# Quantus-Network/qp-zk-circuits

Measured on AMD Instinct MI355X. Metric: Wormhole proofs/sec, higher is better.
Workload: dtype u64

## Files before the change

### qp-zk-circuits_amd/csrc/poseidon.hpp

```cpp
#pragma once
#include <stddef.h>
#include "gl64.hpp"

namespace poseidon {
using gl::u32;
using gl::u64;

constexpr int WIDTH = 12, RATE = 8, HALF_FULL = 4, PARTIAL = 22, ROUNDS = 30;

GL_HD u64 sbox7(u64 x) {
    u64 x2 = gl::sqr(x), x4 = gl::sqr(x2), x3 = gl::mul(x, x2);
    return gl::mul(x3, x4);
}
#if defined(__HIP_DEVICE_COMPILE__) && defined(POSEIDON_GROUPED_SBOX)
template <int N>
__device__ __forceinline__ void sbox7_layer(u64 (&x)[N]) {
    u64 x2[N], x3[N], x4[N];
    gl::mul_group(x2, x, x);
    gl::mul_group(x4, x2, x2);
    gl::mul_group(x3, x, x2);
    gl::mul_group(x, x3, x4);
}
__device__ __forceinline__ u64 sbox7_lane(u64 x) {
    u64 a[1] = {x}, x2[1];
    gl::mul_group(x2, a, a);
    u64 l[2] = {x2[0], x}, r[2] = {x2[0], x2[0]}, q[2];
    gl::mul_group(q, l, r);
    u64 c[1] = {q[0]}, d[1] = {q[1]}, o[1];
    gl::mul_group(o, c, d);
    return o[0];
}
#else
template <int N>
GL_HD void sbox7_layer(u64 (&x)[N]) {
#if defined(__HIP_DEVICE_COMPILE__)
#pragma unroll
#endif
    for (int i = 0; i < N; i++) x[i] = sbox7(x[i]);
}
GL_HD u64 sbox7_lane(u64 x) { return sbox7(x); }
#endif

GL_HD void mds_layer_naive(u64 (&s)[WIDTH]) {
    constexpr u32 C[WIDTH] = {17, 15, 41, 16, 2, 28, 13, 13, 39, 18, 34, 20};
    u32 lo[WIDTH], hi[WIDTH];
#pragma unroll
    for (int i = 0; i < WIDTH; i++) { lo[i] = (u32)s[i]; hi[i] = (u32)(s[i] >> 32); }
#pragma unroll
    for (int r = 0; r < WIDTH; r++) {
        u64 al = 0, ah = 0;
#pragma unroll
        for (int i = 0; i < WIDTH; i++) {
            const int j = (i + r) % WIDTH;
            al += (u64)lo[j] * C[i];
            ah += (u64)hi[j] * C[i];
        }
        if (r == 0) { al += (u64)lo[0] * 8u; ah += (u64)hi[0] * 8u; }
        u64 low = al + (ah << 32);
        u32 top = (u32)(ah >> 32) + (low < al ? 1u : 0u);
        s[r] = gl::reduce96(low, top);
    }
}

typedef long long i64;
GL_HD i64 shl(i64 x, int k) { return (i64)((u64)x << k); }
GL_HD void mds_circulant_half(const i64 (&x)[WIDTH], i64 (&o)[WIDTH]) {
    i64 U1[3], Um[3], F[3], H[3];
#pragma unroll
    for (int b = 0; b < 3; b++) {
        const i64 e = x[b] + x[b + 6], f = x[b] - x[b + 6], g = x[b + 3] + x[b + 9], h = x[b + 3] - x[b + 9];
        U1[b] = e + g; Um[b] = e - g; F[b] = f; H[b] = h;
    }
    const i64 T = U1[0] + U1[1] + U1[2];
    const i64 A[3] = {T + U1[2], T + U1[0], T + U1[1]};
    const i64 B[3] = {shl(Um[2], 3) - Um[0] - shl(Um[1], 1),
                      -(shl(Um[0], 3) + Um[1] + shl(Um[2], 1)),
                      shl(Um[0], 1) - shl(Um[1], 3) - Um[2]};
    const i64 f0 = F[0], f1 = F[1], f2 = F[2], h0 = H[0], h1 = H[1], h2 = H[2];
    const i64 R[3] = {shl(f0, 1) - h0 + f1 - shl(h1, 4) + f2 + shl(h2, 2),
                      -shl(f0, 2) + h0 + shl(f1, 1) - h1 + f2 - shl(h2, 4),
                      shl(f0, 4) + h0 - shl(f1, 2) + h1 + shl(f2, 1) - h2};
    const i64 I[3] = {f0 + shl(h0, 1) + shl(f1, 4) + h1 - shl(f2, 2) + h2,
                      -f0 - shl(h0, 2) + f1 + shl(h1, 1) + shl(f2, 4) + h2,
                      -f0 + shl(h0, 4) - f1 - shl(h1, 2) + f2 + shl(h2, 1)};
#pragma unroll
    for (int b = 0; b < 3; b++) {
        const i64 a16 = shl(A[b], 4), p = a16 + B[b], q = a16 - B[b];
        o[b] = p + R[b]; o[b + 3] = q + I[b]; o[b + 6] = p - R[b]; o[b + 9] = q - I[b];
    }
}

template <int FIRST, int COUNT>
GL_HD void mds_layer_rows(u64 (&s)[WIDTH]) {
    static_assert(FIRST >= 0 && COUNT >= 1 && FIRST + COUNT <= WIDTH, "rows of the state");
    i64 lo[WIDTH], hi[WIDTH], ol[WIDTH], oh[WIDTH];
#pragma unroll
    for (int i = 0; i < WIDTH; i++) { lo[i] = (i64)(u32)s[i]; hi[i] = (i64)(s[i] >> 32); }
    mds_circulant_half(lo, ol);
    mds_circulant_half(hi, oh);
    ol[0] += shl(lo[0], 3); oh[0] += shl(hi[0], 3);
#pragma unroll
    for (int r = FIRST; r < FIRST + COUNT; r++) {
        const u64 al = (u64)ol[r], ah = (u64)oh[r];
        const u64 low = al + (ah << 32);
        const u32 top = (u32)(ah >> 32) + (low < al ? 1u : 0u);
        s[r] = gl::reduce96(low, top);
    }
}
GL_HD void mds_layer(u64 (&s)[WIDTH]) { mds_layer_rows<0, WIDTH>(s); }

struct Spectrum { i64 U1[3], Um[3], F[3], H[3]; };
GL_HD void spectrum_of(const i64 (&x)[WIDTH], Spectrum &s) {
#pragma unroll
    for (int b = 0; b < 3; b++) {
        const i64 e = x[b] + x[b + 6], g = x[b + 3] + x[b + 9];
        s.U1[b] = e + g; s.Um[b] = e - g; s.F[b] = x[b] - x[b + 6]; s.H[b] = x[b + 3] - x[b + 9];
    }
}
GL_HD void spectrum_times_circulant(Spectrum &s) {
    const i64 T = s.U1[0] + s.U1[1] + s.U1[2];
    const i64 A0 = T + s.U1[2], A1 = T + s.U1[0], A2 = T + s.U1[1];
    const i64 B0 = shl(s.Um[2], 3) - s.Um[0] - shl(s.Um[1], 1);
    const i64 B1 = -(shl(s.Um[0], 3) + s.Um[1] + shl(s.Um[2], 1));
    const i64 B2 = shl(s.Um[0], 1) - shl(s.Um[1], 3) - s.Um[2];
    const i64 f0 = s.F[0], f1 = s.F[1], f2 = s.F[2], h0 = s.H[0], h1 = s.H[1], h2 = s.H[2];
    const i64 R0 = shl(f0, 1) - h0 + f1 - shl(h1, 4) + f2 + shl(h2, 2);
    const i64 R1 = -shl(f0, 2) + h0 + shl(f1, 1) - h1 + f2 - shl(h2, 4);
    const i64 R2 = shl(f0, 4) + h0 - shl(f1, 2) + h1 + shl(f2, 1) - h2;
    const i64 I0 = f0 + shl(h0, 1) + shl(f1, 4) + h1 - shl(f2, 2) + h2;
    const i64 I1 = -f0 - shl(h0, 2) + f1 + shl(h1, 1) + shl(f2, 4) + h2;
    const i64 I2 = -f0 + shl(h0, 4) - f1 - shl(h1, 2) + f2 + shl(h2, 1);
    s.U1[0] = shl(A0, 6); s.U1[1] = shl(A1, 6); s.U1[2] = shl(A2, 6);
    s.Um[0] = shl(B0, 2); s.Um[1] = shl(B1, 2); s.Um[2] = shl(B2, 2);
    s.F[0] = shl(R0, 1); s.F[1] = shl(R1, 1); s.F[2] = shl(R2, 1);
    s.H[0] = shl(I0, 1); s.H[1] = shl(I1, 1); s.H[2] = shl(I2, 1);
}
GL_HD i64 spectrum_lane0(const Spectrum &s) { return (s.U1[0] + s.Um[0] + shl(s.F[0], 1)) >> 2; }
GL_HD void vector_of(const Spectrum &s, i64 (&x)[WIDTH]) {
#pragma unroll
    for (int b = 0; b < 3; b++) {
        const i64 p = s.U1[b] + s.Um[b], q = s.U1[b] - s.Um[b], f2 = shl(s.F[b], 1), h2 = shl(s.H[b], 1);
        x[b] = (p + f2) >> 2; x[b + 6] = (p - f2) >> 2; x[b + 3] = (q + h2) >> 2; x[b + 9] = (q - h2) >> 2;
    }
}
GL_HD u64 join_halves(i64 lo, i64 hi) {
    const u64 al = (u64)lo, ah = (u64)hi;
    const u64 low = al + (ah << 32);
    const u32 top = (u32)(ah >> 32) + (low < al ? 1u : 0u);
    return gl::reduce96(low, top);
}
GL_HD void renormalize_pair(i64 &lo, i64 &hi) {
    const i64 k = (lo >> 32) & ~(i64)3;
    lo -= shl(k, 32); hi += k;
    const i64 m = (hi >> 32) & ~(i64)3;
    hi -= shl(m, 32); hi += m; lo -= m;
}
GL_HD void renormalize(Spectrum &sl, Spectrum &sh) {
#pragma unroll
    for (int b = 0; b < 3; b++) {
        renormalize_pair(sl.U1[b], sh.U1[b]); renormalize_pair(sl.Um[b], sh.Um[b]);
        renormalize_pair(sl.F[b], sh.F[b]); renormalize_pair(sl.H[b], sh.H[b]);
    }
}
GL_HD u64 join_signed_halves(i64 lo, i64 hi) { return join_halves(lo + (((i64)1 << 60) + ((i64)1 << 28)), hi + (((i64)1 << 60) - ((i64)1 << 29))); }

GL_HD void partial_rounds_spectral(u64 (&s)[WIDTH], const u64 *rc0) {
    i64 lo[WIDTH], hi[WIDTH];
#pragma unroll
    for (int i = 0; i < WIDTH; i++) { lo[i] = (i64)(u32)s[i]; hi[i] = (i64)(s[i] >> 32); }
    Spectrum sl, sh;
    spectrum_of(lo, sl); spectrum_of(hi, sh);
    i64 x_lo = lo[0], x_hi = hi[0];
    i64 d_lo = 0, d_hi = 0;
    u64 x0 = s[0];
#pragma unroll 1
    for (int k0 = 0; k0 < PARTIAL; k0 += 3) {
#pragma unroll
        for (int kk = 0; kk < 3; kk++) {
            const int k = k0 + kk;
            if (k < PARTIAL) {
                if (k) x0 = join_signed_halves(x_lo + d_lo, x_hi + d_hi);
                const u64 y = sbox7_lane(gl::add_canonical(x0, rc0[k * WIDTH]));
                const i64 y_lo = (i64)(u32)y, y_hi = (i64)(y >> 32);
                const i64 in_lo = y_lo - x_lo, in_hi = y_hi - x_hi;
                sl.U1[0] += in_lo; sl.Um[0] += in_lo; sl.F[0] += in_lo;
                sh.U1[0] += in_hi; sh.Um[0] += in_hi; sh.F[0] += in_hi;
                spectrum_times_circulant(sl); spectrum_times_circulant(sh);
                d_lo = shl(y_lo, 3); d_hi = shl(y_hi, 3);
                if (kk == 2 && k + 1 < PARTIAL) renormalize(sl, sh);
                x_lo = spectrum_lane0(sl); x_hi = spectrum_lane0(sh);
            }
        }
    }
    vector_of(sl, lo); vector_of(sh, hi);
    lo[0] += d_lo; hi[0] += d_hi;
#pragma unroll
    for (int i = 0; i < WIDTH; i++) s[i] = join_signed_halves(lo[i], hi[i]);
}

GL_HD void permute(u64 (&s)[WIDTH], const u64 *rc) {
    int r = 0;
    for (int k = 0; k < HALF_FULL; k++, r++) {
#pragma unroll
        for (int i = 0; i < WIDTH; i++) s[i] = gl::add_canonical(s[i], rc[r * WIDTH + i]);
        sbox7_layer(s);
        mds_layer(s);
    }
#pragma unroll
    for (int i = 1; i < WIDTH; i++) s[i] = gl::add_canonical(s[i], rc[r * WIDTH + i]);
    partial_rounds_spectral(s, rc + r * WIDTH);
    r += PARTIAL;
    for (int k = 0; k < HALF_FULL; k++, r++) {
#pragma unroll
        for (int i = 0; i < WIDTH; i++) s[i] = gl::add_canonical(s[i], rc[r * WIDTH + i]);
        sbox7_layer(s);
        mds_layer(s);
    }
#pragma unroll
    for (int i = 0; i < WIDTH; i++) s[i] = gl::canon(s[i]);
}
GL_HD void permute_layerwise(u64 (&s)[WIDTH], const u64 *rc) {
    int r = 0;
    for (int k = 0; k < HALF_FULL; k++, r++) {
#pragma unroll
        for (int i = 0; i < WIDTH; i++) s[i] = sbox7(gl::add_canonical(s[i], rc[r * WIDTH + i]));
        mds_layer(s);
    }
#pragma unroll
    for (int i = 1; i < WIDTH; i++) s[i] = gl::add_canonical(s[i], rc[r * WIDTH + i]);
    for (int k = 0; k < PARTIAL; k++, r++) {
        s[0] = sbox7(gl::add_canonical(s[0], rc[r * WIDTH]));
        mds_layer(s);
    }
    for (int k = 0; k < HALF_FULL; k++, r++) {
#pragma unroll
        for (int i = 0; i < WIDTH; i++) s[i] = sbox7(gl::add_canonical(s[i], rc[r * WIDTH + i]));
        mds_layer(s);
    }
#pragma unroll
    for (int i = 0; i < WIDTH; i++) s[i] = gl::canon(s[i]);
}
GL_HD void permute_textbook(u64 (&s)[WIDTH], const u64 *rc) {
    int r = 0;
    for (int k = 0; k < ROUNDS; k++, r++) {
        const bool full = k < HALF_FULL || k >= HALF_FULL + PARTIAL;
        for (int i = 0; i < WIDTH; i++) s[i] = gl::add_canonical(s[i], rc[r * WIDTH + i]);
        for (int i = 0; i < (full ? WIDTH : 1); i++) s[i] = sbox7(s[i]);
        mds_layer_naive(s);
    }
    for (int i = 0; i < WIDTH; i++) s[i] = gl::canon(s[i]);
}

constexpr int FP_FIRST = 0, FP_RC = 12, FP_VS = 34, FP_WHATS = FP_VS + 22 * 11, FP_INIT = FP_WHATS + 22 * 11, FP_WORDS = FP_INIT + 121;
constexpr u64 MDS_00 = 25;

GL_HD void fast_partial_enter(u64 (&s)[WIDTH], const u64 *fp) {
#pragma unroll
    for (int i = 0; i < WIDTH; i++) s[i] = gl::add(s[i], fp[FP_FIRST + i]);
    u64 t[11];
    for (int c = 0; c < 11; c++) {
        u64 acc = 0;
        for (int r = 0; r < 11; r++) acc = gl::add(acc, gl::mul(fp[FP_INIT + c * 11 + r], s[1 + r]));
        t[c] = acc;
    }
    for (int c = 0; c < 11; c++) s[1 + c] = t[c];
}
GL_HD void fast_partial_linear(u64 (&s)[WIDTH], const u64 *fp, int r) {
    const u64 s0 = gl::add(s[0], fp[FP_RC + r]);
    u64 d = gl::mul(s0, MDS_00);
    for (int i = 0; i < 11; i++) d = gl::add(d, gl::mul(fp[FP_WHATS + r * 11 + i], s[1 + i]));
    for (int i = 0; i < 11; i++) s[1 + i] = gl::add(s[1 + i], gl::mul(s0, fp[FP_VS + r * 11 + i]));
    s[0] = d;
}
const u64 *host_fast_partial();

void derive_round_constants(u64 *out360);
const u64 *host_round_constants();
const u64 *host_hash_round_constants();

}

namespace poseidon2 {
using gl::u64;
struct Params {
    u64 rc_ext[8 * 12];
    u64 rc_int[22];
    u64 diag_m1[12];
    u64 m4[16];
};
constexpr int PARAM_WORDS = 96 + 22 + 12 + 16;
const Params &qp_params();

GL_HD void ext_layer(u64 (&s)[12], const Params &p) {
    u64 t[12];
#pragma unroll
    for (int b = 0; b < 3; b++)
#pragma unroll
        for (int i = 0; i < 4; i++) {
            u64 acc = 0;
#pragma unroll
            for (int j = 0; j < 4; j++) acc = gl::add(acc, gl::mul(p.m4[4 * i + j], s[4 * b + j]));
            t[4 * b + i] = acc;
        }
#pragma unroll
    for (int i = 0; i < 4; i++) {
        const u64 sum = gl::add(gl::add(t[i], t[4 + i]), t[8 + i]);
#pragma unroll
        for (int b = 0; b < 3; b++) s[4 * b + i] = gl::add(t[4 * b + i], sum);
    }
}
GL_HD void ext_layer_qp(u64 (&s)[12]) {
    u64 t[12];
#pragma unroll
    for (int b = 0; b < 3; b++) {
        const u64 a = s[4 * b], bb = s[4 * b + 1], c = s[4 * b + 2], d = s[4 * b + 3];
        const u64 sum = gl::add(gl::add(a, bb), gl::add(c, d));
        t[4 * b] = gl::add(gl::add(sum, a), gl::add(bb, bb));
        t[4 * b + 1] = gl::add(gl::add(sum, bb), gl::add(c, c));
        t[4 * b + 2] = gl::add(gl::add(sum, c), gl::add(d, d));
        t[4 * b + 3] = gl::add(gl::add(sum, d), gl::add(a, a));
    }
#pragma unroll
    for (int i = 0; i < 4; i++) {
        const u64 sum = gl::add(gl::add(t[i], t[4 + i]), t[8 + i]);
#pragma unroll
        for (int b = 0; b < 3; b++) s[4 * b + i] = gl::add(t[4 * b + i], sum);
    }
}
GL_HD void int_layer(u64 (&s)[12], const Params &p) {
    u64 sum = 0;
#pragma unroll
    for (int i = 0; i < 12; i++) sum = gl::add(sum, s[i]);
#pragma unroll
    for (int i = 0; i < 12; i++) s[i] = gl::add(gl::mul(s[i], p.diag_m1[i]), sum);
}
GL_HD void permute_qp(u64 (&s)[12], const Params &p) {
    ext_layer_qp(s);
    for (int r = 0; r < 4; r++) {
#pragma unroll
        for (int i = 0; i < 12; i++) s[i] = gl::add_canonical(s[i], p.rc_ext[r * 12 + i]);
        poseidon::sbox7_layer(s);
        ext_layer_qp(s);
    }
    for (int r = 0; r < 22; r++) {
        s[0] = poseidon::sbox7_lane(gl::add_canonical(s[0], p.rc_int[r]));
        int_layer(s, p);
    }
    for (int r = 4; r < 8; r++) {
#pragma unroll
        for (int i = 0; i < 12; i++) s[i] = gl::add_canonical(s[i], p.rc_ext[r * 12 + i]);
        poseidon::sbox7_layer(s);
        ext_layer_qp(s);
    }
#pragma unroll
    for (int i = 0; i < 12; i++) s[i] = gl::canon(s[i]);
}
GL_HD void permute(u64 (&s)[12], const Params &p) {
    ext_layer(s, p);
    for (int r = 0; r < 4; r++) {
#pragma unroll
        for (int i = 0; i < 12; i++) s[i] = gl::add(s[i], p.rc_ext[r * 12 + i]);
        poseidon::sbox7_layer(s);
        ext_layer(s, p);
    }
    for (int r = 0; r < 22; r++) {
        s[0] = poseidon::sbox7_lane(gl::add(s[0], p.rc_int[r]));
        int_layer(s, p);
    }
    for (int r = 4; r < 8; r++) {
#pragma unroll
        for (int i = 0; i < 12; i++) s[i] = gl::add(s[i], p.rc_ext[r * 12 + i]);
        poseidon::sbox7_layer(s);
        ext_layer(s, p);
    }
#pragma unroll
    for (int i = 0; i < 12; i++) s[i] = gl::canon(s[i]);
}
}

namespace hasher {
enum Kind : int { POSEIDON = 0, POSEIDON2 = 1 };
struct Config {
    int kind = POSEIDON;
    poseidon2::Params p2{};
    void permute(gl::u64 (&s)[12]) const;
};
const Config &process_default();
void set_process_default(int kind, const poseidon2::Params *p);
inline int kind() { return process_default().kind; }
inline void host_permute(gl::u64 (&s)[12]) { process_default().permute(s); }
inline void hash_no_pad(const Config &h, const gl::u64 *in, size_t n, gl::u64 out[4]) {
    gl::u64 st[12] = {0};
    for (size_t i = 0; i < n; i += 8) {
        for (size_t k = 0; k < 8 && i + k < n; k++) st[k] = gl::canon(in[i + k]);
        h.permute(st);
    }
    for (int i = 0; i < 4; i++) out[i] = st[i];
}
}
```

### qp-zk-circuits_amd/csrc/poseidon_mfma.hpp

```cpp
#pragma once
#include <string.h>
#include <utility>
#include "poseidon.hpp"

namespace pmf {
using gl::u32;
using gl::u64;
#if defined(__HIPCC__)
typedef int v4i __attribute__((ext_vector_type(4)));
typedef int v16i __attribute__((ext_vector_type(16)));
#endif

constexpr int LIMBS = 8, N_GROUP = 6, N_FIN = 3, FIN_STEPS = 9, N_ELEM = 36;
constexpr int group_steps(int g) { return 3 + g; }
constexpr int group_base(int g) { int b = 0; for (int i = 0; i < g; i++) b += group_steps(i); return b; }
constexpr int N_GROUP_TILES = group_base(N_GROUP);
constexpr int N_TILES = N_GROUP_TILES + N_FIN * FIN_STEPS;
constexpr int CINIT_OFF = N_TILES * 1024;
constexpr int G_OFF = CINIT_OFF + (N_GROUP + N_FIN) * 128;
constexpr int TABLE_BYTES = G_OFF + 32;
static_assert(N_GROUP_TILES == 33 && TABLE_BYTES % 16 == 0, "table layout");
constexpr u64 DIGIT_BIAS = 0x8080808080808080ull;

constexpr u64 mds_entry(int r, int j) {
    constexpr u32 C[12] = {17, 15, 41, 16, 2, 28, 13, 13, 39, 18, 34, 20};
    return C[(j - r + 12) % 12] + ((r == 0 && j == 0) ? 8 : 0);
}
constexpr u64 small_g(int d) {
    u64 R[12] = {1, 0, 0, 0, 0, 0, 0, 0, 0, 0, 0, 0};
    for (int it = 0; it < d; it++) {
        u64 T[12] = {};
        for (int j = 1; j < 12; j++)
            for (int i = 0; i < 12; i++) T[j] += R[i] * mds_entry(i, j);
        for (int j = 0; j < 12; j++) R[j] = T[j];
    }
    u64 g = 0;
    for (int i = 0; i < 12; i++) g += R[i] * mds_entry(i, 0);
    return g;
}
constexpr u32 G0 = (u32)small_g(0), G1 = (u32)small_g(1), G2 = (u32)small_g(2);
static_assert(small_g(0) == 25 && small_g(1) < small_g(2) && small_g(2) < (1ull << 21), "group coefficients: the bound of reduce96_terms");

GL_HD u64 to_digits(u64 v) {
    u64 t = v + DIGIT_BIAS;
    t += (t < v) ? 0xFFFFFFFFull : 0ull;
    return t ^ DIGIT_BIAS;
}
GL_HD u32 byte_perm(u32 s0, u32 s1, u32 sel) {
#if defined(__HIP_DEVICE_COMPILE__)
    return __builtin_amdgcn_perm(s0, s1, sel);
#else
    const u64 pool = ((u64)s0 << 32) | s1;
    u32 r = 0;
    for (int i = 0; i < 4; i++) r |= (u32)((pool >> (8 * ((sel >> (8 * i)) & 7))) & 0xFF) << (8 * i);
    return r;
#endif
}
GL_HD void recombine_wide(const u32 (&z)[LIMBS], u64 &lo, u32 &top) {
    const u32 a0 = (z[3] << 24) | z[0], a1 = byte_perm(z[6], z[3], 0x05040201u), a2 = z[6] >> 16;
    const u32 b0 = z[1] << 8, b1 = (z[7] << 24) | z[4], b2 = z[7] >> 8;
    const u32 c0 = z[2] << 16, c1 = byte_perm(z[5], z[2], 0x06050402u);
    typedef unsigned __int128 u128;
    const u128 A = ((u128)a2 << 64) | ((u128)a1 << 32) | a0;
    const u128 B = ((u128)b2 << 64) | ((u128)b1 << 32) | b0;
    const u128 Cc = ((u128)c1 << 32) | c0;
    const u128 S = A + B + Cc;
    lo = (u64)S; top = (u32)(S >> 64);
}
GL_HD u64 recombine(const u32 (&z)[LIMBS]) {
    u64 lo; u32 top;
    recombine_wide(z, lo, top);
    return gl::reduce96(lo, top);
}
constexpr int MAX_GROUP_TERMS = 3;
GL_HD u64 reduce96_terms(u64 lo, u32 top, const u64 *y, const u32 *g, int n) {
    if (n == 0) return gl::reduce96(lo, top);
    u64 al = (u32)lo, ah = ((u64)top << 32) | (lo >> 32);
#if defined(__HIP_DEVICE_COMPILE__)
#pragma unroll
#endif
    for (int i = 0; i < n; i++) { al += (u64)(u32)y[i] * g[i]; ah += (y[i] >> 32) * g[i]; }
    const u64 low = al + (ah << 32);
    return gl::reduce96(low, (u32)(ah >> 32) + (low < al ? 1u : 0u));
}
constexpr int row_of(int output, int limb) { const int i = 8 * (output & 1) + limb; return (i & 3) + 8 * (i >> 2) + 4 * (output >> 1); }

#if !defined(__HIP_DEVICE_COMPILE__)
namespace host {
typedef unsigned __int128 u128;
inline u64 fmul(u64 a, u64 b) { return (u64)((u128)a * b % gl::P); }
inline u64 fadd(u64 a, u64 b) { return (u64)(((u128)a + b) % gl::P); }
inline u64 fsub(u64 a, u64 b) { return (u64)(((u128)a + gl::P - b % gl::P) % gl::P); }
inline bool const_digits(u64 w, signed char (&d)[LIMBS]) {
    w %= gl::P;
    __int128 rep = w <= 0x7F7F7F7F7F7F7F7Full ? (__int128)w : (__int128)w - (__int128)gl::P;
    for (int a = 0; a < LIMBS; a++) {
        int dg = (int)(rep & 255);
        if (dg >= 128) dg -= 256;
        d[a] = (signed char)dg;
        rep = (rep - dg) / 256;
    }
    return rep == 0;
}
struct Rows { u64 w[4][N_ELEM]; u64 addc[4]; };
inline bool fill_tiles(const Rows &rw, int steps, unsigned char *tiles, unsigned char *cinit) {
    static signed char dig[4][N_ELEM][8][LIMBS];
    for (int o = 0; o < 4; o++)
        for (int e = 0; e < N_ELEM; e++) {
            u64 w = rw.w[o][e] % gl::P;
            for (int b = 0; b < 8; b++) { if (!const_digits(w, dig[o][e][b])) return false; w = fmul(w, 256); }
        }
    for (int q = 0; q < steps; q++)
        for (int o = 0; o < 4; o++)
            for (int limb = 0; limb < LIMBS; limb++)
                for (int k = 0; k < 32; k++) {
                    const int lane = row_of(o, limb) + 32 * (k >> 4), j = k & 15, e = 4 * q + (k >> 3), b = k & 7;
                    tiles[(size_t)q * 1024 + lane * 16 + j] = (unsigned char)dig[o][e][b][limb];
                }
    u64 bias = 0, pw = 1u << 23;
    for (int l = 0; l < LIMBS; l++) { bias = fadd(bias, pw); pw = fmul(pw, 256); }
    for (int h = 0; h < 2; h++)
        for (int i = 0; i < 16; i++) {
            const u64 c = fsub(rw.addc[2 * h + (i >> 3)], bias);
            const u32 v = (1u << 23) + (u32)((c >> (8 * (i & 7))) & 0xFF);
            memcpy(cinit + h * 64 + i * 4, &v, 4);
        }
    return true;
}
struct Linear {
    u64 M[12][12], pre[12][12];
    u64 rc[22][12], after[12];
};
inline bool build_tables(const Linear &L, unsigned char *tab) {
    static u64 R[23][12], G[22], Q[22][12], NP[12][12];
    const auto &M = L.M;
    for (int j = 0; j < 12; j++) R[0][j] = j == 0;
    for (int k = 0; k < 22; k++)
        for (int j = 0; j < 12; j++) {
            u64 a = 0;
            if (j >= 1) for (int i = 0; i < 12; i++) a = fadd(a, fmul(R[k][i], M[i][j]));
            R[k + 1][j] = a;
        }
    for (int d = 0; d < 22; d++) { u64 a = 0; for (int i = 0; i < 12; i++) a = fadd(a, fmul(R[d][i], M[i][0])); G[d] = a; }
    for (int i = 0; i < 12; i++) Q[0][i] = M[i][0] % gl::P;
    for (int d = 0; d + 1 < 22; d++)
        for (int i = 0; i < 12; i++) { u64 a = 0; for (int j = 1; j < 12; j++) a = fadd(a, fmul(M[i][j], Q[d][j])); Q[d + 1][i] = a; }
    for (int i = 0; i < 12; i++) for (int j = 0; j < 12; j++) NP[i][j] = i == j;
    for (int it = 0; it < 22; it++) {
        u64 T[12][12];
        for (int i = 0; i < 12; i++) for (int e = 0; e < 12; e++) { u64 a = 0; for (int j = 1; j < 12; j++) a = fadd(a, fmul(M[i][j], NP[j][e])); T[i][e] = a; }
        memcpy(NP, T, sizeof T);
    }
    static u64 accv[23][12];
    memset(accv, 0, sizeof accv);
    for (int k = 0; k < 22; k++)
        for (int i = 0; i < 12; i++) { u64 a = 0; for (int j = 1; j < 12; j++) a = fadd(a, fmul(M[i][j], fadd(accv[k][j], L.rc[k][j] % gl::P))); accv[k + 1][i] = a; }
    memset(tab, 0, TABLE_BYTES);
    for (int g = 0; g < N_GROUP; g++) {
        Rows rw{};
        for (int o = 0; o < 4; o++) {
            const int k = 4 * g + o;
            if (k >= 22) continue;
            for (int e = 0; e < 12; e++) { u64 a = 0; for (int i = 0; i < 12; i++) a = fadd(a, fmul(R[k][i], L.pre[i][e])); rw.w[o][e] = a; }
            for (int j = 0; j < 4 * g; j++) rw.w[o][12 + j] = G[k - 1 - j];
            rw.addc[o] = fadd(accv[k][0], L.rc[k][0] % gl::P);
        }
        if (!fill_tiles(rw, group_steps(g), tab + (size_t)group_base(g) * 1024, tab + CINIT_OFF + g * 128)) return false;
    }
    for (int f = 0; f < N_FIN; f++) {
        Rows rw{};
        for (int o = 0; o < 4; o++) {
            const int i = 4 * f + o;
            for (int e = 0; e < 12; e++) { u64 a = 0; for (int j = 0; j < 12; j++) a = fadd(a, fmul(NP[i][j], L.pre[j][e])); rw.w[o][e] = a; }
            for (int j = 0; j < 22; j++) rw.w[o][12 + j] = Q[21 - j][i];
            rw.addc[o] = fadd(accv[22][i], L.after[i] % gl::P);
        }
        if (!fill_tiles(rw, FIN_STEPS, tab + (size_t)(N_GROUP_TILES + f * FIN_STEPS) * 1024, tab + CINIT_OFF + (N_GROUP + f) * 128)) return false;
    }
    memcpy(tab + G_OFF, G, 3 * sizeof(u64));
    return true;
}
inline bool build_tables(const u64 *rc, unsigned char *tab) {
    static Linear L;
    memset(&L, 0, sizeof L);
    for (int r = 0; r < 12; r++) for (int j = 0; j < 12; j++) L.M[r][j] = L.pre[r][j] = mds_entry(r, j);
    for (int k = 0; k < 22; k++) L.rc[k][0] = rc[(4 + k) * 12];
    for (int i = 1; i < 12; i++) L.rc[0][i] = rc[4 * 12 + i];
    for (int i = 0; i < 12; i++) L.after[i] = rc[26 * 12 + i];
    if (!build_tables(L, tab)) return false;
    u64 g[3]; memcpy(g, tab + G_OFF, sizeof g);
    return g[0] == G0 && g[1] == G1 && g[2] == G2;
}
inline bool build_tables_gate(const u64 *rcp, unsigned char *tab) {
    static Linear L;
    memset(&L, 0, sizeof L);
    for (int r = 0; r < 12; r++) for (int j = 0; j < 12; j++) L.M[r][j] = L.pre[r][j] = mds_entry(r, j);
    for (int k = 0; k < 22; k++) for (int i = 0; i < 12; i++) L.rc[k][i] = rcp[(4 + k) * 12 + i];
    for (int i = 0; i < 12; i++) L.after[i] = rcp[26 * 12 + i];
    return build_tables(L, tab);
}
inline bool build_tables_p2(const poseidon2::Params &p, unsigned char *tab) {
    static Linear L;
    memset(&L, 0, sizeof L);
    for (int j = 0; j < 12; j++) {
        u64 e[12] = {}, f[12] = {};
        e[j] = f[j] = 1;
        poseidon2::int_layer(e, p); poseidon2::ext_layer_qp(f);
        for (int i = 0; i < 12; i++) { L.M[i][j] = gl::canon(e[i]); L.pre[i][j] = gl::canon(f[i]); }
    }
    for (int k = 0; k < 22; k++) L.rc[k][0] = p.rc_int[k];
    for (int i = 0; i < 12; i++) L.after[i] = p.rc_ext[4 * 12 + i];
    return build_tables(L, tab);
}
inline bool emu_gemm(const unsigned char *tab, int tile0, int cidx, int steps, const u64 *D, u32 (&Z)[4][LIMBS]) {
    for (int o = 0; o < 4; o++)
        for (int limb = 0; limb < LIMBS; limb++) {
            const int row = row_of(o, limb);
            u32 c; memcpy(&c, tab + CINIT_OFF + cidx * 128 + (o >> 1) * 64 + (8 * (o & 1) + limb) * 4, 4);
            long long acc = c;
            for (int q = 0; q < steps; q++)
                for (int k = 0; k < 32; k++) {
                    const int lane = row + 32 * (k >> 4), j = k & 15;
                    const int a = (signed char)tab[(size_t)(tile0 + q) * 1024 + lane * 16 + j];
                    const int bdig = (signed char)(D[4 * q + (k >> 3)] >> (8 * (k & 7)));
                    acc += (long long)a * bdig;
                }
            if (acc < 0 || acc >= (1 << 24)) return false;
            Z[o][limb] = (u32)acc;
        }
    return true;
}
inline bool emu_partial_rounds(u64 (&s)[12], const unsigned char *tab) {
    u64 D[N_ELEM] = {}, y[24], G[3];
    memcpy(G, tab + G_OFF, sizeof G);
    const bool small = G[0] == G0 && G[1] == G1 && G[2] == G2;
    for (int e = 0; e < 12; e++) D[e] = to_digits(s[e]);
    for (int g = 0; g < N_GROUP; g++) {
        u32 Z[4][LIMBS];
        if (!emu_gemm(tab, group_base(g), g, group_steps(g), D, Z)) return false;
        for (int o = 0; o < 4 && 4 * g + o < 22; o++) {
            const int k = 4 * g + o;
            u64 x;
            if (small) {
                u64 lo; u32 top, gg[MAX_GROUP_TERMS];
                recombine_wide(Z[o], lo, top);
                for (int i = 0; i < o; i++) gg[i] = (u32)G[o - 1 - i];
                x = reduce96_terms(lo, top, y + 4 * g, gg, o);
            } else {
                x = recombine(Z[o]);
                for (int j = 4 * g; j < k; j++) x = gl::add(x, gl::mul(y[j], G[k - 1 - j]));
            }
            y[k] = poseidon::sbox7_lane(x);
        }
        for (int o = 0; o < 4 && 4 * g + o < 22; o++) D[12 + 4 * g + o] = to_digits(y[4 * g + o]);
    }
    for (int f = 0; f < N_FIN; f++) {
        u32 Z[4][LIMBS];
        if (!emu_gemm(tab, N_GROUP_TILES + f * FIN_STEPS, N_GROUP + f, FIN_STEPS, D, Z)) return false;
        for (int o = 0; o < 4; o++) s[4 * f + o] = recombine(Z[o]);
    }
    return true;
}
inline bool emu_permute_textbook(u64 (&s)[12], const u64 *rcp, const unsigned char *tab) {
    using namespace poseidon;
    int r = 0;
    for (int k = 0; k < HALF_FULL; k++, r++) {
        for (int i = 0; i < WIDTH; i++) s[i] = sbox7(gl::add_canonical(s[i], rcp[r * WIDTH + i]));
        if (k + 1 < HALF_FULL) mds_layer(s);
    }
    if (!emu_partial_rounds(s, tab)) return false;
    r += 1 + PARTIAL;
    for (int i = 0; i < WIDTH; i++) s[i] = sbox7(s[i]);
    mds_layer(s);
    for (int k = 1; k < HALF_FULL; k++, r++) {
        for (int i = 0; i < WIDTH; i++) s[i] = sbox7(gl::add_canonical(s[i], rcp[r * WIDTH + i]));
        mds_layer(s);
    }
    for (int i = 0; i < WIDTH; i++) s[i] = gl::canon(s[i]);
    return true;
}
inline bool emu_permute(u64 (&s)[12], const u64 *rc, const unsigned char *tab) {
    using namespace poseidon;
    int r = 0;
    for (int k = 0; k < HALF_FULL; k++, r++) {
        for (int i = 0; i < WIDTH; i++) s[i] = gl::add_canonical(s[i], rc[r * WIDTH + i]);
        sbox7_layer(s);
        if (k + 1 < HALF_FULL) mds_layer(s);
    }
    if (!emu_partial_rounds(s, tab)) return false;
    r += 1 + PARTIAL;
    sbox7_layer(s); mds_layer(s);
    for (int k = 1; k < HALF_FULL; k++, r++) {
        for (int i = 0; i < WIDTH; i++) s[i] = gl::add_canonical(s[i], rc[r * WIDTH + i]);
        sbox7_layer(s);
        mds_layer(s);
    }
    for (int i = 0; i < WIDTH; i++) s[i] = gl::canon(s[i]);
    return true;
}
inline bool emu_permute_p2(u64 (&s)[12], const poseidon2::Params &p, const unsigned char *tab) {
    poseidon2::ext_layer_qp(s);
    for (int r = 0; r < 4; r++) {
        for (int i = 0; i < 12; i++) s[i] = gl::add(s[i], p.rc_ext[r * 12 + i]);
        poseidon::sbox7_layer(s);
        if (r < 3) poseidon2::ext_layer_qp(s);
    }
    if (!emu_partial_rounds(s, tab)) return false;
    poseidon::sbox7_layer(s); poseidon2::ext_layer_qp(s);
    for (int r = 5; r < 8; r++) {
        for (int i = 0; i < 12; i++) s[i] = gl::add(s[i], p.rc_ext[r * 12 + i]);
        poseidon::sbox7_layer(s);
        poseidon2::ext_layer_qp(s);
    }
    for (int i = 0; i < 12; i++) s[i] = gl::canon(s[i]);
    return true;
}
template <class F, class Gf>
inline bool selfcheck_with(F plain, Gf emu, int n) {
    u64 seed = 0x243F6A8885A308D3ull;
    for (int t = 0; t < n; t++) {
        u64 a[12], b[12];
        for (int i = 0; i < 12; i++) {
            seed = seed * 6364136223846793005ull + 1442695040888963407ull;
            u64 v = seed ^ (seed >> 29);
            if (t % 7 == 0) v = (i & 1) ? ~0ull - (v & 0xFF) : (v & 0xFF);
            if (t % 11 == 0) v = gl::P - 1 - (v & 3);
            a[i] = b[i] = v;
        }
        plain(a);
        if (!emu(b)) return false;
        for (int i = 0; i < 12; i++) if (a[i] != b[i]) return false;
    }
    return true;
}
inline bool selfcheck(const u64 *rc, const unsigned char *tab, int n = 2000) {
    return selfcheck_with([&](u64 (&s)[12]) { poseidon::permute(s, rc); }, [&](u64 (&s)[12]) { return emu_permute(s, rc, tab); }, n);
}
inline bool selfcheck_gate(const u64 *rcp, const unsigned char *tab, int n = 2000) {
    return selfcheck_with([&](u64 (&s)[12]) { for (int i = 0; i < 12; i++) s[i] = gl::canon(s[i]); poseidon::permute_textbook(s, rcp); },
                          [&](u64 (&s)[12]) { for (int i = 0; i < 12; i++) s[i] = gl::canon(s[i]); return emu_permute_textbook(s, rcp, tab); }, n);
}
inline bool selfcheck_p2(const poseidon2::Params &p, const unsigned char *tab, int n = 2000) {
    return selfcheck_with([&](u64 (&s)[12]) { poseidon2::permute_qp(s, p); }, [&](u64 (&s)[12]) { return emu_permute_p2(s, p, tab); }, n);
}
}
inline bool build_tables(const u64 *rc, unsigned char *tab) { return host::build_tables(rc, tab); }
inline bool host_selfcheck(const u64 *rc, const unsigned char *tab, int n = 2000) { return host::selfcheck(rc, tab, n); }
inline bool build_tables_gate(const u64 *rcp, unsigned char *tab) { return host::build_tables_gate(rcp, tab); }
inline bool host_selfcheck_gate(const u64 *rcp, const unsigned char *tab, int n = 2000) { return host::selfcheck_gate(rcp, tab, n); }
inline bool build_tables_p2(const poseidon2::Params &p, unsigned char *tab) { return host::build_tables_p2(p, tab); }
inline bool host_selfcheck_p2(const poseidon2::Params &p, const unsigned char *tab, int n = 2000) { return host::selfcheck_p2(p, tab, n); }
#else
bool build_tables(const u64 *, unsigned char *);
bool host_selfcheck(const u64 *, const unsigned char *, int n = 2000);
bool build_tables_p2(const poseidon2::Params &, unsigned char *);
bool build_tables_gate(const u64 *, unsigned char *);
bool host_selfcheck_gate(const u64 *, const unsigned char *, int n = 2000);
bool host_selfcheck_p2(const poseidon2::Params &, const unsigned char *, int n = 2000);
#endif

#if defined(__HIP_DEVICE_COMPILE__)
__device__ __forceinline__ void swap32(u32 &x, u32 &y) {
    auto r = __builtin_amdgcn_permlane32_swap(x, y, false, false);
    x = r[0]; y = r[1];
}
struct Run {
    u32 Dlo[N_ELEM], Dhi[N_ELEM];
    v4i B0[FIN_STEPS], B1[FIN_STEPS];
    u64 y[24];
    u64 Gd[3];
    const unsigned char *lds;
};
__device__ __forceinline__ void form_step(Run &st, int q) {
    swap32(st.Dlo[4 * q], st.Dlo[4 * q + 2]); swap32(st.Dhi[4 * q], st.Dhi[4 * q + 2]);
    swap32(st.Dlo[4 * q + 1], st.Dlo[4 * q + 3]); swap32(st.Dhi[4 * q + 1], st.Dhi[4 * q + 3]);
    st.B0[q] = v4i{(int)st.Dlo[4 * q], (int)st.Dhi[4 * q], (int)st.Dlo[4 * q + 1], (int)st.Dhi[4 * q + 1]};
    st.B1[q] = v4i{(int)st.Dlo[4 * q + 2], (int)st.Dhi[4 * q + 2], (int)st.Dlo[4 * q + 3], (int)st.Dhi[4 * q + 3]};
}
template <int STEPS>
__device__ __forceinline__ void gemm(const Run &st, int tile0, int cidx, u32 (&Z)[4][LIMBS]) {
    const int lane = threadIdx.x & 63;
    const v4i *cp = (const v4i *)(st.lds + CINIT_OFF + cidx * 128 + (lane >> 5) * 64);
    v16i a0, a1;
#pragma unroll
    for (int i = 0; i < 4; i++) {
        const v4i c = cp[i];
        a0[4 * i] = c[0]; a0[4 * i + 1] = c[1]; a0[4 * i + 2] = c[2]; a0[4 * i + 3] = c[3];
    }
    a1 = a0;
    const v4i *ap = (const v4i *)(st.lds + (size_t)tile0 * 1024) + lane;
#pragma unroll
    for (int q = 0; q < STEPS; q++) {
        const v4i a = ap[q * 64];
        a0 = __builtin_amdgcn_mfma_i32_32x32x32_i8(a, st.B0[q], a0, 0, 0, 0);
        a1 = __builtin_amdgcn_mfma_i32_32x32x32_i8(a, st.B1[q], a1, 0, 0, 0);
    }
#ifndef PMF_NO_KEEPALIVE
    asm volatile("" : "+v"(a0), "+v"(a1));
#endif
#pragma unroll
    for (int i = 0; i < 16; i++) {
        u32 x = (u32)a0[i], yv = (u32)a1[i];
        swap32(x, yv);
        Z[i >> 3][i & 7] = x; Z[2 + (i >> 3)][i & 7] = yv;
    }
}
struct SboxOfInput { __device__ __forceinline__ u64 operator()(int, u64 x) const { return poseidon::sbox7_lane(x); } };
template <int G, bool SMALL_G, class F>
__device__ __forceinline__ void group_step(Run &st, F &f) {
    u32 Z[4][LIMBS];
    gemm<group_steps(G)>(st, group_base(G), G, Z);
    constexpr int n = 4 * G + 4 <= 22 ? 4 : 22 - 4 * G;
#pragma unroll
    for (int o = 0; o < n; o++) {
        const int k = 4 * G + o;
        u64 x;
        if constexpr (SMALL_G) {
            constexpr u32 Gc[3] = {G0, G1, G2};
            u64 lo, yy[MAX_GROUP_TERMS] = {};
            u32 top, gg[MAX_GROUP_TERMS] = {};
            recombine_wide(Z[o], lo, top);
#pragma unroll
            for (int i = 0; i < o; i++) { yy[i] = st.y[4 * G + i]; gg[i] = Gc[o - 1 - i]; }
            x = reduce96_terms(lo, top, yy, gg, o);
        } else {
            x = recombine(Z[o]);
#pragma unroll
            for (int j = 4 * G; j < k; j++) x = gl::add(x, gl::mul(st.y[j], st.Gd[k - 1 - j]));
        }
        st.y[k] = f(k, x);
    }
#pragma unroll
    for (int o = 0; o < n; o++) {
        const u64 t = to_digits(st.y[4 * G + o]);
        st.Dlo[12 + 4 * G + o] = (u32)t; st.Dhi[12 + 4 * G + o] = (u32)(t >> 32);
    }
    form_step(st, 3 + G);
}
template <bool SMALL_G, class F, int... G>
__device__ __forceinline__ void all_groups(Run &st, F &f, std::integer_sequence<int, G...>) { (group_step<G, SMALL_G>(st, f), ...); }

template <bool SMALL_G, class F>
__device__ __forceinline__ void partial_rounds(u64 (&s)[12], const unsigned char *lds, F &f) {
    Run st;
    st.lds = lds;
    if (!SMALL_G) {
#pragma unroll
        for (int d = 0; d < 3; d++) {
            const u64 g = *(const u64 *)(lds + G_OFF + 8 * d);
            st.Gd[d] = ((u64)(u32)__builtin_amdgcn_readfirstlane((int)(g >> 32)) << 32) | (u32)__builtin_amdgcn_readfirstlane((int)(u32)g);
        }
    }
#pragma unroll
    for (int e = 0; e < N_ELEM; e++) {
        const u64 t = e < 12 ? to_digits(s[e]) : 0;
        st.Dlo[e] = (u32)t; st.Dhi[e] = (u32)(t >> 32);
    }
    form_step(st, 0); form_step(st, 1); form_step(st, 2);
    all_groups<SMALL_G>(st, f, std::make_integer_sequence<int, N_GROUP>{});
#pragma unroll
    for (int f = 0; f < N_FIN; f++) {
        u32 Z[4][LIMBS];
        gemm<FIN_STEPS>(st, N_GROUP_TILES + f * FIN_STEPS, N_GROUP + f, Z);
#pragma unroll
        for (int o = 0; o < 4; o++) s[4 * f + o] = recombine(Z[o]);
    }
}
__device__ __forceinline__ void permute_head(u64 (&s)[12], const u64 *rc, const unsigned char *lds) {
    using namespace poseidon;
    int r = 0;
    for (int k = 0; k < HALF_FULL; k++, r++) {
#pragma unroll
        for (int i = 0; i < WIDTH; i++) s[i] = gl::add_canonical(s[i], rc[r * WIDTH + i]);
        sbox7_layer(s);
        if (k + 1 < HALF_FULL) mds_layer(s);
    }
    SboxOfInput f;
    partial_rounds<true>(s, lds, f);
}
__device__ __forceinline__ void permute_tail_rounds(u64 (&s)[12], const u64 *rc) {
    using namespace poseidon;
    int r = HALF_FULL + 1 + PARTIAL;
    for (int k = 1; k < HALF_FULL; k++, r++) {
        sbox7_layer(s);
        mds_layer(s);
#pragma unroll
        for (int i = 0; i < WIDTH; i++) s[i] = gl::add_canonical(s[i], rc[r * WIDTH + i]);
    }
    sbox7_layer(s);
}
template <int FIRST, int COUNT, bool CANON>
__device__ __forceinline__ void last_layer_rows(u64 (&s)[12]) {
    poseidon::mds_layer_rows<FIRST, COUNT>(s);
    if (CANON) {
#pragma unroll
        for (int i = FIRST; i < FIRST + COUNT; i++) s[i] = gl::canon(s[i]);
    }
}
template <int FIRST, int COUNT, bool CANON>
__device__ __forceinline__ void permute_tail_rows(u64 (&s)[12], const u64 *rc) {
    permute_tail_rounds(s, rc);
    last_layer_rows<FIRST, COUNT, CANON>(s);
}
__device__ __forceinline__ void permute_tail(u64 (&s)[12], const u64 *rc) { permute_tail_rows<0, 12, true>(s, rc); }
__device__ __forceinline__ void permute(u64 (&s)[12], const u64 *rc, const unsigned char *lds) {
    permute_head(s, rc, lds);
    permute_tail(s, rc);
}
__device__ __forceinline__ void permute_p2qp(u64 (&s)[12], const poseidon2::Params &p, const unsigned char *lds) {
    poseidon2::ext_layer_qp(s);
    for (int r = 0; r < 4; r++) {
#pragma unroll
        for (int i = 0; i < 12; i++) s[i] = gl::add_canonical(s[i], p.rc_ext[r * 12 + i]);
        poseidon::sbox7_layer(s);
        if (r < 3) poseidon2::ext_layer_qp(s);
    }
    SboxOfInput f;
    partial_rounds<false>(s, lds, f);
    poseidon::sbox7_layer(s);
    poseidon2::ext_layer_qp(s);
    for (int r = 5; r < 8; r++) {
#pragma unroll
        for (int i = 0; i < 12; i++) s[i] = gl::add_canonical(s[i], p.rc_ext[r * 12 + i]);
        poseidon::sbox7_layer(s);
        poseidon2::ext_layer_qp(s);
    }
#pragma unroll
    for (int i = 0; i < 12; i++) s[i] = gl::canon(s[i]);
}
#elif defined(__HIPCC__)
__device__ void permute(u64 (&s)[12], const u64 *rc, const unsigned char *lds);
__device__ void permute_head(u64 (&s)[12], const u64 *rc, const unsigned char *lds);
__device__ void permute_tail(u64 (&s)[12], const u64 *rc);
__device__ void permute_tail_rounds(u64 (&s)[12], const u64 *rc);
template <int FIRST, int COUNT, bool CANON> __device__ void last_layer_rows(u64 (&)[12]) {}
template <int FIRST, int COUNT, bool CANON> __device__ void permute_tail_rows(u64 (&)[12], const u64 *) {}
__device__ void permute_p2qp(u64 (&s)[12], const poseidon2::Params &p, const unsigned char *lds);
template <bool SMALL_G, class F> __device__ void partial_rounds(u64 (&)[12], const unsigned char *, F &) {}
#endif

}
```

Baseline: 1604.

## Compute full-round MDS with wrapping u64 plus 32-bit top-bits transform and fused constants

Replaces the full-round MDS layer, which split each element into 32-bit halves and ran two signed 64-bit circulant transforms. The new version runs the circulant once on wrapping u64 words and once on the 23 top bits in u32, then rebuilds the 96-bit result with a carry check before reduce96. The round-constant addition is folded into that final reduction, so the separate add_canonical pass disappears. This cuts 64-bit integer work per full round, but depends on the bound argument (static_assert) holding for the carry reconstruction.

```diff
diff --git a/qp-zk-circuits_amd/csrc/poseidon.hpp b/qp-zk-circuits_amd/csrc/poseidon.hpp
--- a/qp-zk-circuits_amd/csrc/poseidon.hpp
+++ b/qp-zk-circuits_amd/csrc/poseidon.hpp
@@ -108,6 +108,67 @@
     }
 }
 GL_HD void mds_layer(u64 (&s)[WIDTH]) { mds_layer_rows<0, WIDTH>(s); }
+
+template <class W>
+GL_HD void mds_circulant_wrapping(const W (&x)[WIDTH], W (&o)[WIDTH]) {
+    W U1[3], Um[3], F[3], H[3];
+#if defined(__HIP_DEVICE_COMPILE__)
+#pragma unroll
+#endif
+    for (int b = 0; b < 3; b++) {
+        const W e = x[b] + x[b + 6], g = x[b + 3] + x[b + 9];
+        U1[b] = e + g; Um[b] = e - g; F[b] = x[b] - x[b + 6]; H[b] = x[b + 3] - x[b + 9];
+    }
+    const W T = U1[0] + U1[1] + U1[2];
+    const W A[3] = {T + U1[2], T + U1[0], T + U1[1]};
+    const W B[3] = {(Um[2] << 3) - ((Um[1] << 1) + Um[0]),
+                    (Um[0] << 3) + (Um[2] << 1) + Um[1],
+                    (Um[0] << 1) - ((Um[1] << 3) + Um[2])};
+    const W f0 = F[0], f1 = F[1], f2 = F[2], h0 = H[0], h1 = H[1], h2 = H[2];
+    const W R[3] = {((f0 << 1) + (h2 << 2) + f1 + f2) - ((h1 << 4) + h0),
+                    ((f1 << 1) + h0 + f2) - ((f0 << 2) + (h2 << 4) + h1),
+                    ((f0 << 4) + (f2 << 1) + h0 + h1) - ((f1 << 2) + h2)};
+    const W I[3] = {((h0 << 1) + (f1 << 4) + f0 + h1 + h2) - (f2 << 2),
+                    ((h1 << 1) + (f2 << 4) + f1 + h2) - ((h0 << 2) + f0),
+                    ((h0 << 4) + (h2 << 1) + f2) - ((h1 << 2) + f0 + f1)};
+#if defined(__HIP_DEVICE_COMPILE__)
+#pragma unroll
+#endif
+    for (int b = 0; b < 3; b++) {
+        const W a16 = A[b] << 4;
+        const W p = b == 1 ? a16 - B[b] : a16 + B[b], q = b == 1 ? a16 + B[b] : a16 - B[b];
+        o[b] = p + R[b]; o[b + 3] = q + I[b]; o[b + 6] = p - R[b]; o[b + 9] = q - I[b];
+    }
+}
+template <int FIRST, int COUNT, bool ADD_RC>
+GL_HD void mds_layer_rows_words_rc(u64 (&s)[WIDTH], const u64 *rc) {
+    static_assert(FIRST >= 0 && COUNT >= 1 && FIRST + COUNT <= WIDTH, "rows of the state");
+    constexpr int TOP_SHIFT = 41, TOP_BITS = 64 - TOP_SHIFT;
+    static_assert(265ull * ((1ull << TOP_BITS) - 1) < (1ull << 32), "the top transform, with a constant's top bits, fits 32 bits");
+    u64 ol[WIDTH];
+    u32 t[WIDTH], ot[WIDTH];
+#if defined(__HIP_DEVICE_COMPILE__)
+#pragma unroll
+#endif
+    for (int i = 0; i < WIDTH; i++) t[i] = (u32)(s[i] >> TOP_SHIFT);
+    mds_circulant_wrapping<u64>(s, ol);
+    mds_circulant_wrapping<u32>(t, ot);
+    ol[0] += s[0] << 3; ot[0] += t[0] << 3;
+#if defined(__HIP_DEVICE_COMPILE__)
+#pragma unroll
+#endif
+    for (int r = FIRST; r < FIRST + COUNT; r++) {
+        u64 L = ol[r];
+        u32 Ht = ot[r];
+        if (ADD_RC) { L += rc[r]; Ht += (u32)(rc[r] >> TOP_SHIFT); }
+        const u32 carry = (u32)(L >> 32) < (Ht << (32 - TOP_BITS)) ? 1u : 0u;
+        s[r] = gl::reduce96(L, (Ht >> TOP_BITS) + carry);
+    }
+}
+template <int FIRST, int COUNT>
+GL_HD void mds_layer_rows_words(u64 (&s)[WIDTH]) { mds_layer_rows_words_rc<FIRST, COUNT, false>(s, nullptr); }
+GL_HD void mds_layer_words_rc(u64 (&s)[WIDTH], const u64 *rc) { mds_layer_rows_words_rc<0, WIDTH, true>(s, rc); }
+GL_HD void mds_layer_words(u64 (&s)[WIDTH]) { mds_layer_rows_words<0, WIDTH>(s); }
 
 struct Spectrum { i64 U1[3], Um[3], F[3], H[3]; };
 GL_HD void spectrum_of(const i64 (&x)[WIDTH], Spectrum &s) {
diff --git a/qp-zk-circuits_amd/csrc/poseidon_mfma.hpp b/qp-zk-circuits_amd/csrc/poseidon_mfma.hpp
--- a/qp-zk-circuits_amd/csrc/poseidon_mfma.hpp
+++ b/qp-zk-circuits_amd/csrc/poseidon_mfma.hpp
@@ -468,12 +468,11 @@
 }
 __device__ __forceinline__ void permute_head(u64 (&s)[12], const u64 *rc, const unsigned char *lds) {
     using namespace poseidon;
-    int r = 0;
-    for (int k = 0; k < HALF_FULL; k++, r++) {
-#pragma unroll
-        for (int i = 0; i < WIDTH; i++) s[i] = gl::add_canonical(s[i], rc[r * WIDTH + i]);
+#pragma unroll
+    for (int i = 0; i < WIDTH; i++) s[i] = gl::add_canonical(s[i], rc[i]);
+    for (int k = 0; k < HALF_FULL; k++) {
         sbox7_layer(s);
-        if (k + 1 < HALF_FULL) mds_layer(s);
+        if (k + 1 < HALF_FULL) mds_layer_words_rc(s, rc + (k + 1) * WIDTH);
     }
     SboxOfInput f;
     partial_rounds<true>(s, lds, f);
@@ -483,15 +482,13 @@
     int r = HALF_FULL + 1 + PARTIAL;
     for (int k = 1; k < HALF_FULL; k++, r++) {
         sbox7_layer(s);
-        mds_layer(s);
-#pragma unroll
-        for (int i = 0; i < WIDTH; i++) s[i] = gl::add_canonical(s[i], rc[r * WIDTH + i]);
+        mds_layer_words_rc(s, rc + r * WIDTH);
     }
     sbox7_layer(s);
 }
 template <int FIRST, int COUNT, bool CANON>
 __device__ __forceinline__ void last_layer_rows(u64 (&s)[12]) {
-    poseidon::mds_layer_rows<FIRST, COUNT>(s);
+    poseidon::mds_layer_rows_words<FIRST, COUNT>(s);
     if (CANON) {
 #pragma unroll
         for (int i = FIRST; i < FIRST + COUNT; i++) s[i] = gl::canon(s[i]);
```

New measurement: 1661 (median of 6 runs). 1.04x the previous value.
